# UBC-AWP/vision-sam3-yolo-lameless

Hardware: AMD Instinct MI355X
Metric: frames/sec (whole node) for YOLO+SAM3+DINOv3 feature extraction, 1080p clips (higher is better)
Workload: dtype f16; 1 GPU; BASELINE cfg#5, dense schedule: fused per-frame path on a synthetic 5 s @ 30 fps 1080p clip (150 unique BGR frames resident in HBM): YOLOv8-l detect (letterbox 384x640, NMS, scale_boxes; f16 plan) -> SAM (Hiera-B+ image encoder + FPN at 1024x1024, box-prompted mask decoder, 1080p mask + statistics + contour features) + DINOv3 ViT-L/16 embed (224x224) on EVERY frame; per-frame records packed, gathe; parallelism=one clip per GPU, 1 GPU(s), one gather per step, streams=7

## Files before the change

### vision-sam3-yolo-lameless_amd/csrc/pre.hip

```cpp
#include "common.h"

namespace {

constexpr int PRECISION_BITS = 32 - 8 - 2;

__device__ __forceinline__ uint8_t clip8(int v) {
  const int top = (256 << PRECISION_BITS) - 1;
  v = v < 0 ? 0 : (v > top ? top : v);
  return (uint8_t)((unsigned)v >> PRECISION_BITS);
}

__device__ __forceinline__ int tap(unsigned byte, int coef) { return __mul24((int)byte, coef); }

constexpr int RESIZE_H_MAX_ROW = 16384;
constexpr int RESIZE_H_LDS = 2 * RESIZE_H_MAX_ROW;
constexpr int RESIZE_H_ROWS = 4;

inline int resize_h_group(int rowb) {
  int r = (RESIZE_H_LDS - 16) / rowb;
  r = r > 8 ? 8 : r;
  return r >= RESIZE_H_ROWS ? r / RESIZE_H_ROWS * RESIZE_H_ROWS : r;
}

__global__ __launch_bounds__(256) void pil_resize_h_kernel(const uint8_t* __restrict__ src, uint8_t* __restrict__ dst,
                                                           int n, int sh, int sw, int dw, int group,
                                                           const int32_t* __restrict__ bounds,
                                                           const int32_t* __restrict__ kk, int ksize, int swap_rb) {
  __shared__ __attribute__((aligned(16))) uint8_t buf[RESIZE_H_LDS];
  const int rowb = sw * 3;
  const int64_t rows = (int64_t)n * sh;
  const int dwq = (dw + 3) & ~3;
  for (int64_t row0 = (int64_t)blockIdx.x * group; row0 < rows; row0 += (int64_t)gridDim.x * group) {
    const int nr = rows - row0 < group ? (int)(rows - row0) : group;
    const uint8_t* s0 = src + row0 * rowb;
    const int span = nr * rowb;
    const int mis = (int)(reinterpret_cast<uintptr_t>(s0) & 15);
    int head = mis ? 16 - mis : 0;
    head = head > span ? span : head;
    for (int i = threadIdx.x; i < head; i += blockDim.x) buf[mis + i] = s0[i];
    const int nvec = (span - head) / 16;
    for (int v = threadIdx.x; v < nvec; v += blockDim.x)
      *reinterpret_cast<u32x4*>(buf + mis + head + v * 16) = *reinterpret_cast<const u32x4*>(s0 + head + v * 16);
    for (int i = head + nvec * 16 + threadIdx.x; i < span; i += blockDim.x) buf[mis + i] = s0[i];
    __syncthreads();
    const int ntask = dwq * ((nr + RESIZE_H_ROWS - 1) / RESIZE_H_ROWS);
    for (int t0 = 0; t0 < ntask; t0 += blockDim.x) {
      const int t = t0 + threadIdx.x;
      const int rg = t / dwq, xq = t - rg * dwq;
      const int r0 = rg * RESIZE_H_ROWS;
      const bool live = t < ntask && xq < dw;
      const int xo = xq < dw ? xq : dw - 1;
      int rb[RESIZE_H_ROWS];
#pragma unroll
      for (int r = 0; r < RESIZE_H_ROWS; ++r) rb[r] = mis + (r0 + r < nr ? r0 + r : nr - 1) * rowb;
      const int xmin = bounds[2 * xo], cnt = bounds[2 * xo + 1];
      const int32_t* k = kk + (int64_t)xo * ksize;
      int a[RESIZE_H_ROWS][3];
#pragma unroll
      for (int r = 0; r < RESIZE_H_ROWS; ++r) a[r][0] = a[r][1] = a[r][2] = 1 << (PRECISION_BITS - 1);
      for (int x = 0; x < cnt; ++x) {
        const int c = k[x];
        const int off = (xmin + x) * 3;
#pragma unroll
        for (int r = 0; r < RESIZE_H_ROWS; ++r) {
          const uint8_t* s = buf + rb[r] + off;
          a[r][0] += tap(s[0], c);
          a[r][1] += tap(s[1], c);
          a[r][2] += tap(s[2], c);
        }
      }
      const int j = xq & 3;
      const bool quad = xq - j + 4 <= dw;
#pragma unroll
      for (int r = 0; r < RESIZE_H_ROWS; ++r) {
        const unsigned b0 = clip8(swap_rb ? a[r][2] : a[r][0]), b1 = clip8(a[r][1]), b2 = clip8(swap_rb ? a[r][0] : a[r][2]);
        const unsigned px = b0 | (b1 << 8) | (b2 << 16);
        const unsigned nx = __shfl_down(px, 1, 64);
        if (!live || r0 + r >= nr) continue;
        uint8_t* d = dst + (row0 + r0 + r) * dw * 3 + xq * 3;
        if (quad && ((reinterpret_cast<uintptr_t>(d) - 3 * j) & 3) == 0) {
          if (j < 3) *reinterpret_cast<unsigned*>(d - 3 * j + 4 * j) = (px >> (8 * j)) | (nx << (24 - 8 * j));
        } else {
          d[0] = (uint8_t)b0;
          d[1] = (uint8_t)b1;
          d[2] = (uint8_t)b2;
        }
      }
    }
    __syncthreads();
  }
}

__global__ __launch_bounds__(256) void pil_resize_v_kernel(const uint8_t* __restrict__ src, uint8_t* __restrict__ dst,
                                                           int n, int sh, int dh, int w,
                                                           const int32_t* __restrict__ bounds,
                                                           const int32_t* __restrict__ kk, int ksize) {
  const int rowb = w * 3;
  const int64_t total = (int64_t)n * dh * rowb;
  for (int64_t i = (int64_t)blockIdx.x * blockDim.x + threadIdx.x; i < total; i += (int64_t)gridDim.x * blockDim.x) {
    const int xb = (int)(i % rowb);
    const int64_t r = i / rowb;
    const int yo = (int)(r % dh);
    const int img = (int)(r / dh);
    const int ymin = bounds[2 * yo], cnt = bounds[2 * yo + 1];
    const int32_t* k = kk + (int64_t)yo * ksize;
    const uint8_t* s = src + ((int64_t)img * sh + ymin) * rowb + xb;
    int a = 1 << (PRECISION_BITS - 1);
    for (int y = 0; y < cnt; ++y) a += tap(s[(int64_t)y * rowb], k[y]);
    dst[i] = clip8(a);
  }
}

template <int DW>
__global__ __launch_bounds__(256) void pil_resize_vw_kernel(const uint8_t* __restrict__ src, uint8_t* __restrict__ dst, int n, int sh,
                                                            int dh, int w, const int32_t* __restrict__ bounds,
                                                            const int32_t* __restrict__ kk, int ksize) {
  typedef unsigned vec_t __attribute__((ext_vector_type(DW)));
  const int rowb = w * 3, roww = (rowb + 4 * DW - 1) / (4 * DW);
  const int64_t total = (int64_t)n * dh * roww;
  for (int64_t i = (int64_t)blockIdx.x * blockDim.x + threadIdx.x; i < total; i += (int64_t)gridDim.x * blockDim.x) {
    const int xw = (int)(i % roww);
    const int64_t r = i / roww;
    const int yo = (int)(r % dh);
    const int img = (int)(r / dh);
    const int ymin = bounds[2 * yo], cnt = bounds[2 * yo + 1];
    const int32_t* k = kk + (int64_t)yo * ksize;
    const int xb = xw * (4 * DW) + 4 * DW <= rowb ? xw * (4 * DW) : rowb - 4 * DW;
    const uint8_t* s = src + ((int64_t)img * sh + ymin) * rowb + xb;
    int a[4 * DW];
#pragma unroll
    for (int e = 0; e < 4 * DW; ++e) a[e] = 1 << (PRECISION_BITS - 1);
    for (int y = 0; y < cnt; ++y) {
      vec_t v;
      if (DW == 4)
        v = *reinterpret_cast<const vec_t*>(s + (int64_t)y * rowb);
      else
        __builtin_memcpy(&v, s + (int64_t)y * rowb, sizeof(v));
      const int c = k[y];
#pragma unroll
      for (int q = 0; q < DW; ++q) {
        a[4 * q + 0] += tap(v[q] & 255u, c);
        a[4 * q + 1] += tap((v[q] >> 8) & 255u, c);
        a[4 * q + 2] += tap((v[q] >> 16) & 255u, c);
        a[4 * q + 3] += tap(v[q] >> 24, c);
      }
    }
    vec_t o;
#pragma unroll
    for (int q = 0; q < DW; ++q)
      o[q] = (unsigned)clip8(a[4 * q]) | ((unsigned)clip8(a[4 * q + 1]) << 8) | ((unsigned)clip8(a[4 * q + 2]) << 16) |
             ((unsigned)clip8(a[4 * q + 3]) << 24);
    if (DW == 4)
      *reinterpret_cast<vec_t*>(dst + r * rowb + xb) = o;
    else
      __builtin_memcpy(dst + r * rowb + xb, &o, sizeof(o));
  }
}

__global__ __launch_bounds__(256) void patchify_norm_kernel(const uint8_t* __restrict__ img, half_t* __restrict__ out,
                                                            int n, int ih, int iw, int top, int left, int gh, int gw,
                                                            int P, int64_t ldo, const float* __restrict__ lut) {
  const int ch = gh * P, cw = gw * P;
  const int64_t total = (int64_t)n * ch * cw;
  for (int64_t i = (int64_t)blockIdx.x * blockDim.x + threadIdx.x; i < total; i += (int64_t)gridDim.x * blockDim.x) {
    const int x = (int)(i % cw);
    const int64_t r = i / cw;
    const int y = (int)(r % ch);
    const int b = (int)(r / ch);
    const uint8_t* s = img + (((int64_t)b * ih + top + y) * iw + left + x) * 3;
    const int py = y / P, ky = y - py * P, px = x / P, kx = x - px * P;
    half_t* d = out + (((int64_t)b * gh + py) * gw + px) * ldo + (ky * P + kx) * 3;
#pragma unroll
    for (int c = 0; c < 3; ++c) d[c] = (half_t)lut[c * 256 + s[c]];
  }
}

constexpr int FR_ROWS = 8;
constexpr int FR_COLS = 256;
constexpr int FR_MAX_LDS = 65536;

__global__ __launch_bounds__(FR_COLS) void float_resize_patchify_kernel(
    const uint8_t* __restrict__ src, half_t* __restrict__ out, int sh, int sw, int gh, int gw, int P, int64_t ldo,
    const int32_t* __restrict__ bh, const float* __restrict__ kh, int ksh, const int32_t* __restrict__ bv,
    const float* __restrict__ kv, int ksv, int seg_cols, float rescale, float m0, float m1, float m2, float s0, float s1,
    float s2, int swap_rb) {
  extern __shared__ __attribute__((aligned(16))) float seg[];
  const int tid = threadIdx.x;
  const int dh = gh * P, dw = gw * P;
  const int img = blockIdx.z;
  const int x0 = blockIdx.x * FR_COLS, xo = x0 + tid;
  const int y0 = blockIdx.y * FR_ROWS;
  const bool live = xo < dw;
  const int xl = (x0 + FR_COLS < dw ? x0 + FR_COLS : dw) - 1;
  int c_lo = bh[2 * x0];
  c_lo = c_lo < 0 ? 0 : (c_lo > sw ? sw : c_lo);
  int c_hi = bh[2 * xl] + bh[2 * xl + 1];
  c_hi = c_hi > sw ? sw : c_hi;
  if (c_hi > c_lo + seg_cols) c_hi = c_lo + seg_cols;
  if (c_hi < c_lo) c_hi = c_lo;
  int xmin = 0, xcnt = 0;
  if (live) {
    xmin = bh[2 * xo];
    xcnt = bh[2 * xo + 1];
    if (xmin < c_lo) xmin = c_lo;
    if (xcnt > ksh) xcnt = ksh;
    if (xcnt > c_hi - xmin) xcnt = c_hi - xmin;
    if (xcnt < 0) xcnt = 0;
  }
  const float* kx = kh + (int64_t)(live ? xo : 0) * ksh;
  int ymin[FR_ROWS], ycnt[FR_ROWS];
  int r_lo = sh, r_hi = 0;
#pragma unroll
  for (int r = 0; r < FR_ROWS; ++r) {
    ymin[r] = 0;
    ycnt[r] = 0;
    if (y0 + r < dh) {
      int a = bv[2 * (y0 + r)], c = bv[2 * (y0 + r) + 1];
      a = a < 0 ? 0 : a;
      c = c > ksv ? ksv : c;
      c = c > sh - a ? sh - a : c;
      c = c < 0 ? 0 : c;
      ymin[r] = a;
      ycnt[r] = c;
      if (c > 0) {
        r_lo = a < r_lo ? a : r_lo;
        r_hi = a + c > r_hi ? a + c : r_hi;
      }
    }
  }
  float acc[FR_ROWS][3];
#pragma unroll
  for (int r = 0; r < FR_ROWS; ++r) acc[r][0] = acc[r][1] = acc[r][2] = 0.f;

  const int nbytes = (c_hi - c_lo) * 3;
  for (int y = r_lo; y < r_hi; ++y) {
    const uint8_t* srow = src + (((int64_t)img * sh + y) * sw + c_lo) * 3;
    const int mis = (int)(reinterpret_cast<uintptr_t>(srow) & 15);
    int head = mis ? 16 - mis : 0;
    head = head > nbytes ? nbytes : head;
    const int pad = (4 - (head & 3)) & 3;
    float* s = seg + pad;
    if (tid < head) s[tid] = (float)srow[tid] * rescale;
    const int nvec = (nbytes - head) / 16;
    for (int v = tid; v < nvec; v += FR_COLS) {
      const u32x4 x = *reinterpret_cast<const u32x4*>(srow + head + v * 16);
      f32x4* d = reinterpret_cast<f32x4*>(s + head + v * 16);
#pragma unroll
      for (int q = 0; q < 4; ++q) {
        f32x4 f;
        f[0] = (float)(x[q] & 255u) * rescale;
        f[1] = (float)((x[q] >> 8) & 255u) * rescale;
        f[2] = (float)((x[q] >> 16) & 255u) * rescale;
        f[3] = (float)(x[q] >> 24) * rescale;
        d[q] = f;
      }
    }
    for (int i = head + nvec * 16 + tid; i < nbytes; i += FR_COLS) s[i] = (float)srow[i] * rescale;
    __syncthreads();
    float h0 = 0.f, h1 = 0.f, h2 = 0.f;
    const float* p = s + (xmin - c_lo) * 3;
    for (int j = 0; j < xcnt; ++j) {
      const float w = kx[j];
      h0 = __builtin_fmaf(p[3 * j + 0], w, h0);
      h1 = __builtin_fmaf(p[3 * j + 1], w, h1);
      h2 = __builtin_fmaf(p[3 * j + 2], w, h2);
    }
#pragma unroll
    for (int r = 0; r < FR_ROWS; ++r) {
      if (y >= ymin[r] && y < ymin[r] + ycnt[r]) {
        const float w = kv[(int64_t)(y0 + r) * ksv + (y - ymin[r])];
        acc[r][0] = __builtin_fmaf(h0, w, acc[r][0]);
        acc[r][1] = __builtin_fmaf(h1, w, acc[r][1]);
        acc[r][2] = __builtin_fmaf(h2, w, acc[r][2]);
      }
    }
    __syncthreads();
  }
  if (!live) return;
  const int px = xo / P, kxp = xo - px * P;
#pragma unroll
  for (int r = 0; r < FR_ROWS; ++r) {
    const int yo = y0 + r;
    if (yo >= dh) break;
    const int py = yo / P, ky = yo - py * P;
    half_t* d = out + (((int64_t)img * gh + py) * gw + px) * ldo + (ky * P + kxp) * 3;
    d[0] = (half_t)(((swap_rb ? acc[r][2] : acc[r][0]) - m0) / s0);
    d[1] = (half_t)((acc[r][1] - m1) / s1);
    d[2] = (half_t)(((swap_rb ? acc[r][0] : acc[r][2]) - m2) / s2);
  }
}

inline int grid_for(int64_t total) {
  int64_t g = (total + 255) / 256;
  if (g > 256 * 8) g = 256 * 8;
  if (g < 1) g = 1;
  return (int)g;
}

}

extern "C" int lmx_k_pil_resize_h(const uint8_t* src, uint8_t* dst, int n, int sh, int sw, int dw, const int32_t* bounds,
                                  const int32_t* kk, int ksize, int swap_rb, lmx_stream_t stream) {
  LMX_REQUIRE(src && dst && bounds && kk, "lmx_k_pil_resize_h: null pointer");
  LMX_REQUIRE(n > 0 && sh > 0 && sw > 0 && dw > 0 && ksize > 0, "lmx_k_pil_resize_h: shape");
  LMX_REQUIRE(sw * 3 <= RESIZE_H_MAX_ROW, "lmx_k_pil_resize_h: source rows wider than %d pixels are not staged", RESIZE_H_MAX_ROW / 3);
  const int group = resize_h_group(sw * 3);
  const int64_t groups = ((int64_t)n * sh + group - 1) / group;
  hipLaunchKernelGGL(pil_resize_h_kernel, dim3((unsigned)(groups < 256 * 16 ? groups : 256 * 16)), dim3(256), 0,
                     reinterpret_cast<hipStream_t>(stream), src, dst, n, sh, sw, dw, group, bounds, kk, ksize, swap_rb);
  return lmx_launch_check("pil_resize_h_kernel");
}

extern "C" int lmx_k_pil_resize_v(const uint8_t* src, uint8_t* dst, int n, int sh, int dh, int w, const int32_t* bounds,
                                  const int32_t* kk, int ksize, lmx_stream_t stream) {
  LMX_REQUIRE(src && dst && bounds && kk, "lmx_k_pil_resize_v: null pointer");
  LMX_REQUIRE(n > 0 && sh > 0 && dh > 0 && w > 0 && ksize > 0, "lmx_k_pil_resize_v: shape");
  const uintptr_t al = (uintptr_t)src | (uintptr_t)dst | (uintptr_t)(w * 3);
  if ((al & 15) == 0) {
    hipLaunchKernelGGL(pil_resize_vw_kernel<4>, dim3(grid_for((int64_t)n * dh * (w * 3 / 16))), dim3(256), 0,
                       reinterpret_cast<hipStream_t>(stream), src, dst, n, sh, dh, w, bounds, kk, ksize);
    return lmx_launch_check("pil_resize_vw_kernel<4>");
  }
  if (w * 3 >= 4) {
    hipLaunchKernelGGL(pil_resize_vw_kernel<1>, dim3(grid_for((int64_t)n * dh * ((w * 3 + 3) / 4))), dim3(256), 0,
                       reinterpret_cast<hipStream_t>(stream), src, dst, n, sh, dh, w, bounds, kk, ksize);
    return lmx_launch_check("pil_resize_vw_kernel<1>");
  }
  hipLaunchKernelGGL(pil_resize_v_kernel, dim3(grid_for((int64_t)n * dh * w * 3)), dim3(256), 0,
                     reinterpret_cast<hipStream_t>(stream), src, dst, n, sh, dh, w, bounds, kk, ksize);
  return lmx_launch_check("pil_resize_v_kernel");
}

extern "C" int lmx_k_float_resize_patchify(const uint8_t* src, void* out, int n, int sh, int sw, int gh, int gw, int P,
                                           int64_t ldo, const int32_t* bounds_h, const float* kk_h, int ksize_h,
                                           const int32_t* bounds_v, const float* kk_v, int ksize_v, int seg_cols,
                                           float rescale, const float* mean_std, int swap_rb, lmx_stream_t stream) {
  LMX_REQUIRE(src && out && bounds_h && kk_h && bounds_v && kk_v && mean_std, "lmx_k_float_resize_patchify: null pointer");
  LMX_REQUIRE(n > 0 && n <= 65535 && sh > 0 && sw > 0 && gh > 0 && gw > 0 && P > 0 && ksize_h > 0 && ksize_v > 0,
              "lmx_k_float_resize_patchify: shape");
  LMX_REQUIRE(ldo >= (int64_t)P * P * 3, "lmx_k_float_resize_patchify: ldo %lld < P*P*3", (long long)ldo);
  LMX_REQUIRE((int64_t)gh * P <= 65535 * (int64_t)FR_ROWS && (int64_t)gw * P <= (1 << 20), "lmx_k_float_resize_patchify: output size");
  LMX_REQUIRE(seg_cols > 0 && seg_cols <= sw, "lmx_k_float_resize_patchify: seg_cols %d outside 1..%d", seg_cols, sw);
  const int64_t lds = ((int64_t)seg_cols * 3 + 4) * (int64_t)sizeof(float);
  LMX_REQUIRE(lds <= FR_MAX_LDS, "lmx_k_float_resize_patchify: a tile of %d output columns reads %d source columns; more than %d are not staged",
              FR_COLS, seg_cols, (FR_MAX_LDS / 4 - 4) / 3);
  LMX_REQUIRE(mean_std[3] != 0.f && mean_std[4] != 0.f && mean_std[5] != 0.f, "lmx_k_float_resize_patchify: zero std");
  const dim3 grid((unsigned)((gw * P + FR_COLS - 1) / FR_COLS), (unsigned)((gh * P + FR_ROWS - 1) / FR_ROWS), (unsigned)n);
  hipLaunchKernelGGL(float_resize_patchify_kernel, grid, dim3(FR_COLS), (size_t)lds, reinterpret_cast<hipStream_t>(stream), src,
                     reinterpret_cast<half_t*>(out), sh, sw, gh, gw, P, ldo, bounds_h, kk_h, ksize_h, bounds_v, kk_v, ksize_v,
                     seg_cols, rescale, mean_std[0], mean_std[1], mean_std[2], mean_std[3], mean_std[4], mean_std[5], swap_rb);
  return lmx_launch_check("float_resize_patchify_kernel");
}

extern "C" int lmx_k_patchify_norm(const uint8_t* img, void* out, int n, int ih, int iw, int top, int left, int gh,
                                   int gw, int P, int64_t ldo, const float* lut, lmx_stream_t stream) {
  LMX_REQUIRE(img && out && lut, "lmx_k_patchify_norm: null pointer");
  LMX_REQUIRE(n > 0 && gh > 0 && gw > 0 && P > 0 && ldo >= (int64_t)P * P * 3, "lmx_k_patchify_norm: shape");
  LMX_REQUIRE(top >= 0 && left >= 0 && top + gh * P <= ih && left + gw * P <= iw,
              "lmx_k_patchify_norm: crop (%d,%d)+(%d,%d) outside %dx%d", top, left, gh * P, gw * P, ih, iw);
  hipLaunchKernelGGL(patchify_norm_kernel, dim3(grid_for((int64_t)n * gh * P * gw * P)), dim3(256), 0,
                     reinterpret_cast<hipStream_t>(stream), img, reinterpret_cast<half_t*>(out), n, ih, iw, top, left, gh,
                     gw, P, ldo, lut);
  return lmx_launch_check("patchify_norm_kernel");
}
```

### vision-sam3-yolo-lameless_amd/csrc/yolo.hip

```cpp
#include "common.h"

namespace {

inline int grid_for(int64_t total, int block = 256) {
  int64_t g = (total + block - 1) / block;
  if (g > 256 * 8) g = 256 * 8;
  if (g < 1) g = 1;
  return (int)g;
}

__global__ __launch_bounds__(256) void letterbox_kernel(const uint8_t* __restrict__ src, uint8_t* __restrict__ dst, int n,
                                                        int sh, int sw, int rh, int rw, int top, int left, int oh, int ow,
                                                        const int* __restrict__ xofs, const short* __restrict__ ialpha,
                                                        const int* __restrict__ yofs, const short* __restrict__ ibeta,
                                                        int swap_rb, int identity) {
  const int64_t total = (int64_t)n * oh * ow;
  for (int64_t i = (int64_t)blockIdx.x * blockDim.x + threadIdx.x; i < total; i += (int64_t)gridDim.x * blockDim.x) {
    const int ox = (int)(i % ow);
    const int64_t r = i / ow;
    const int oy = (int)(r % oh);
    const int img = (int)(r / oh);
    uint8_t* d = dst + i * 3;
    const int dy = oy - top, dx = ox - left;
    if (dy < 0 || dy >= rh || dx < 0 || dx >= rw) {
      d[0] = d[1] = d[2] = 114;
      continue;
    }
    uint8_t v[3];
    const uint8_t* S = src + (int64_t)img * sh * sw * 3;
    if (identity) {
      const uint8_t* s = S + ((int64_t)dy * sw + dx) * 3;
      v[0] = s[0];
      v[1] = s[1];
      v[2] = s[2];
    } else {
      const int sx0 = xofs[dx];
      const int sx1 = sx0 + 1 < sw ? sx0 + 1 : sw - 1;
      const int a0 = ialpha[2 * dx], a1 = ialpha[2 * dx + 1];
      int sy0 = yofs[dy], sy1 = yofs[dy] + 1;
      sy0 = sy0 < 0 ? 0 : (sy0 < sh ? sy0 : sh - 1);
      sy1 = sy1 < 0 ? 0 : (sy1 < sh ? sy1 : sh - 1);
      const int b0 = ibeta[2 * dy], b1 = ibeta[2 * dy + 1];
      const uint8_t* r0 = S + (int64_t)sy0 * sw * 3;
      const uint8_t* r1 = S + (int64_t)sy1 * sw * 3;
#pragma unroll
      for (int c = 0; c < 3; ++c) {
        const int h0 = (int)r0[sx0 * 3 + c] * a0 + (int)r0[sx1 * 3 + c] * a1;
        const int h1 = (int)r1[sx0 * 3 + c] * a0 + (int)r1[sx1 * 3 + c] * a1;
        const int val = (((b0 * (h0 >> 4)) >> 16) + ((b1 * (h1 >> 4)) >> 16) + 2) >> 2;
        v[c] = (uint8_t)(val < 0 ? 0 : (val > 255 ? 255 : val));
      }
    }
    if (swap_rb) {
      d[0] = v[2];
      d[1] = v[1];
      d[2] = v[0];
    } else {
      d[0] = v[0];
      d[1] = v[1];
      d[2] = v[2];
    }
  }
}

template <int CO_T>
__global__ __launch_bounds__(256) void stem_conv_kernel(const uint8_t* __restrict__ img, const float* __restrict__ w,
                                                        const float* __restrict__ bias, half_t* __restrict__ out, int n,
                                                        int H, int W, int Ho, int Wo, int Cout) {
  extern __shared__ __attribute__((aligned(16))) char smem[];
  float* ws = reinterpret_cast<float*>(smem);
  for (int i = threadIdx.x; i < 27 * Cout; i += blockDim.x) ws[i] = w[i];
  for (int i = threadIdx.x; i < Cout; i += blockDim.x) ws[27 * Cout + i] = bias[i];
  __syncthreads();
  const int64_t total = (int64_t)n * Ho * Wo;
  for (int64_t i = (int64_t)blockIdx.x * blockDim.x + threadIdx.x; i < total; i += (int64_t)gridDim.x * blockDim.x) {
    const int ox = (int)(i % Wo);
    const int64_t r = i / Wo;
    const int oy = (int)(r % Ho);
    const int b = (int)(r / Ho);
    float x[27];
#pragma unroll
    for (int ky = 0; ky < 3; ++ky)
#pragma unroll
      for (int kx = 0; kx < 3; ++kx) {
        const int iy = oy * 2 - 1 + ky, ix = ox * 2 - 1 + kx;
        const bool ok = (unsigned)iy < (unsigned)H && (unsigned)ix < (unsigned)W;
        const uint8_t* s = img + (((int64_t)b * H + (ok ? iy : 0)) * W + (ok ? ix : 0)) * 3;
#pragma unroll
        for (int c = 0; c < 3; ++c) x[(ky * 3 + kx) * 3 + c] = ok ? (float)s[c] / 255.0f : 0.0f;
      }
    half_t* o = out + i * Cout;
    for (int c0 = 0; c0 < Cout; c0 += CO_T) {
      float acc[CO_T];
#pragma unroll
      for (int j = 0; j < CO_T; ++j) acc[j] = ws[27 * Cout + c0 + j];
#pragma unroll
      for (int t = 0; t < 27; ++t) {
        const float xv = x[t];
#pragma unroll
        for (int j = 0; j < CO_T; ++j) acc[j] = fmaf(xv, ws[t * Cout + c0 + j], acc[j]);
      }
      half8_t hv;
#pragma unroll
      for (int j = 0; j < CO_T; ++j) {
        const float v = acc[j] / (1.0f + expf(-acc[j]));
        hv[j] = (half_t)v;
      }
      *reinterpret_cast<half8_t*>(o + c0) = hv;
    }
  }
}

__global__ __launch_bounds__(256) void maxpool5_kernel(const half_t* __restrict__ src, int64_t lds, half_t* __restrict__ dst,
                                                       int64_t ldd, int n, int H, int W, int C) {
  const int cc = C / 8;
  const int64_t total = (int64_t)n * H * W * cc;
  for (int64_t i = (int64_t)blockIdx.x * blockDim.x + threadIdx.x; i < total; i += (int64_t)gridDim.x * blockDim.x) {
    const int c = (int)(i % cc) * 8;
    const int64_t p = i / cc;
    const int x = (int)(p % W);
    const int64_t r = p / W;
    const int y = (int)(r % H);
    const int b = (int)(r / H);
    half8_t m;
#pragma unroll
    for (int e = 0; e < 8; ++e) m[e] = (half_t)(-65504.0f);
    for (int dy = -2; dy <= 2; ++dy) {
      const int yy = y + dy;
      if ((unsigned)yy >= (unsigned)H) continue;
      for (int dx = -2; dx <= 2; ++dx) {
        const int xx = x + dx;
        if ((unsigned)xx >= (unsigned)W) continue;
        const half8_t v = *reinterpret_cast<const half8_t*>(src + (((int64_t)b * H + yy) * W + xx) * lds + c);
#pragma unroll
        for (int e = 0; e < 8; ++e) m[e] = v[e] > m[e] ? v[e] : m[e];
      }
    }
    *reinterpret_cast<half8_t*>(dst + p * ldd + c) = m;
  }
}

__global__ __launch_bounds__(256) void upsample2_kernel(const half_t* __restrict__ src, int64_t lds, half_t* __restrict__ dst,
                                                        int64_t ldd, int n, int H, int W, int C) {
  const int cc = C / 8;
  const int Ho = 2 * H, Wo = 2 * W;
  const int64_t total = (int64_t)n * Ho * Wo * cc;
  for (int64_t i = (int64_t)blockIdx.x * blockDim.x + threadIdx.x; i < total; i += (int64_t)gridDim.x * blockDim.x) {
    const int c = (int)(i % cc) * 8;
    const int64_t p = i / cc;
    const int x = (int)(p % Wo);
    const int64_t r = p / Wo;
    const int y = (int)(r % Ho);
    const int b = (int)(r / Ho);
    *reinterpret_cast<half8_t*>(dst + p * ldd + c) =
        *reinterpret_cast<const half8_t*>(src + (((int64_t)b * H + (y >> 1)) * W + (x >> 1)) * lds + c);
  }
}

__global__ __launch_bounds__(256) void detect_decode_kernel(const float* __restrict__ head, float* __restrict__ pred, int n,
                                                            int H, int W, int nc, int ch, float stride, int a_off,
                                                            int A) {
  const int64_t total = (int64_t)n * H * W * 4;
  for (int64_t i0 = (int64_t)blockIdx.x * blockDim.x; i0 < total; i0 += (int64_t)gridDim.x * blockDim.x) {
    const int64_t i = i0 + threadIdx.x;
    const bool live = i < total;
    const int side = (int)(i & 3);
    const int64_t cell = live ? (i >> 2) : 0;
    const int x = (int)(cell % W);
    const int64_t r = cell / W;
    const int y = (int)(r % H);
    const int b = (int)(r / H);
    const float* hrow = head + cell * ch;
    float l[16];
    float mx = -INFINITY;
#pragma unroll
    for (int k = 0; k < 4; ++k) {
      const f32x4 v = *reinterpret_cast<const f32x4*>(hrow + side * 16 + k * 4);
#pragma unroll
      for (int e = 0; e < 4; ++e) {
        l[k * 4 + e] = v[e];
        mx = fmaxf(mx, v[e]);
      }
    }
    float se = 0.f;
#pragma unroll
    for (int k = 0; k < 16; ++k) {
      l[k] = expf(l[k] - mx);
      se += l[k];
    }
    float dist = 0.f;
#pragma unroll
    for (int k = 0; k < 16; ++k) dist += (l[k] / se) * (float)k;
    const int base = threadIdx.x & ~3;
    const float dl = __shfl(dist, (base & 63) + 0, 64), dt = __shfl(dist, (base & 63) + 1, 64);
    const float dr = __shfl(dist, (base & 63) + 2, 64), db = __shfl(dist, (base & 63) + 3, 64);
    if (!live) continue;
    float* prow = pred + ((int64_t)b * A + a_off + (int64_t)y * W + x) * (4 + nc);
    if (side == 0) {
      const float ax = (float)x + 0.5f, ay = (float)y + 0.5f;
      const float x1 = ax - dl, y1 = ay - dt, x2 = ax + dr, y2 = ay + db;
      prow[0] = ((x1 + x2) / 2.f) * stride;
      prow[1] = ((y1 + y2) / 2.f) * stride;
      prow[2] = (x2 - x1) * stride;
      prow[3] = (y2 - y1) * stride;
    }
    const float* hc = hrow + 64;
    float* pc = prow + 4;
    const bool al = (reinterpret_cast<uintptr_t>(pc) & 15) == 0;
    const int nc4 = nc & ~3;
    for (int c = side * 4; c < nc4; c += 16) {
      const f32x4 v = *reinterpret_cast<const f32x4*>(hc + c);
      f32x4 s;
#pragma unroll
      for (int e = 0; e < 4; ++e) s[e] = 1.0f / (1.0f + expf(-v[e]));
      if (al) {
        *reinterpret_cast<f32x4*>(pc + c) = s;
      } else {
#pragma unroll
        for (int e = 0; e < 4; ++e) pc[c + e] = s[e];
      }
    }
    for (int c = nc4 + side; c < nc; c += 4) pc[c] = 1.0f / (1.0f + expf(-hc[c]));
  }
}

__global__ __launch_bounds__(256) void scale_boxes_kernel(float* __restrict__ boxes, int total, float padx, float pady,
                                                          float gain, float w, float h) {
  const int i = blockIdx.x * blockDim.x + threadIdx.x;
  if (i >= total) return;
  float* b = boxes + (int64_t)i * 4;
  float x1 = (b[0] - padx) / gain, y1 = (b[1] - pady) / gain, x2 = (b[2] - padx) / gain, y2 = (b[3] - pady) / gain;
  b[0] = fminf(fmaxf(x1, 0.f), w);
  b[1] = fminf(fmaxf(y1, 0.f), h);
  b[2] = fminf(fmaxf(x2, 0.f), w);
  b[3] = fminf(fmaxf(y2, 0.f), h);
}

struct PoseLevels {
  const float* raw[3];
  int h[3], w[3], off[3];
  float stride[3];
};
__global__ __launch_bounds__(256) void pose_gather_kernel(const PoseLevels L, int64_t ldk, const int* __restrict__ src,
                                                          const int* __restrict__ counts, int n, int max_det, int K, int ndim,
                                                          float padx, float pady, float gain, float fw, float fh,
                                                          float* __restrict__ out) {
  const int64_t total = (int64_t)n * max_det * K;
  for (int64_t i = (int64_t)blockIdx.x * blockDim.x + threadIdx.x; i < total; i += (int64_t)gridDim.x * blockDim.x) {
    const int k = (int)(i % K);
    const int64_t r = i / K;
    const int j = (int)(r % max_det);
    const int b = (int)(r / max_det);
    float* o = out + i * ndim;
    if (j >= counts[b]) {
      for (int e = 0; e < ndim; ++e) o[e] = 0.f;
      continue;
    }
    const int a = src[(int64_t)b * max_det + j];
    const int l = a >= L.off[2] ? 2 : (a >= L.off[1] ? 1 : 0);
    const int local = a - L.off[l];
    const int y = local / L.w[l], x = local - y * L.w[l];
    const float* v = L.raw[l] + (((int64_t)b * L.h[l] + y) * L.w[l] + x) * ldk + k * ndim;
    const float X = (v[0] * 2.0f + (float)x) * L.stride[l];
    const float Y = (v[1] * 2.0f + (float)y) * L.stride[l];
    o[0] = fminf(fmaxf((X - padx) / gain, 0.f), fw);
    o[1] = fminf(fmaxf((Y - pady) / gain, 0.f), fh);
    if (ndim == 3) o[2] = 1.0f / (1.0f + expf(-v[2]));
  }
}

}

extern "C" int lmx_k_pose_gather(const float* raw0, const float* raw1, const float* raw2, int64_t ldk, const int32_t* hw,
                                 const float* strides, const int32_t* src, const int32_t* counts, int n, int max_det, int K,
                                 int ndim, float padx, float pady, float gain, float w, float h, float* out,
                                 lmx_stream_t stream) {
  LMX_REQUIRE(raw0 && raw1 && raw2 && hw && strides && src && counts && out, "lmx_k_pose_gather: null pointer");
  LMX_REQUIRE(n > 0 && max_det > 0 && K > 0 && (ndim == 2 || ndim == 3) && ldk >= (int64_t)K * ndim && gain > 0.f,
              "lmx_k_pose_gather: arguments");
  PoseLevels L;
  L.raw[0] = raw0;
  L.raw[1] = raw1;
  L.raw[2] = raw2;
  int off = 0;
  for (int l = 0; l < 3; ++l) {
    LMX_REQUIRE(hw[2 * l] > 0 && hw[2 * l + 1] > 0, "lmx_k_pose_gather: level %d geometry", l);
    L.h[l] = hw[2 * l];
    L.w[l] = hw[2 * l + 1];
    L.off[l] = off;
    L.stride[l] = strides[l];
    off += L.h[l] * L.w[l];
  }
  hipLaunchKernelGGL(pose_gather_kernel, dim3(grid_for((int64_t)n * max_det * K)), dim3(256), 0,
                     reinterpret_cast<hipStream_t>(stream), L, ldk, src, counts, n, max_det, K, ndim, padx, pady, gain, w, h, out);
  return lmx_launch_check("pose_gather_kernel");
}

extern "C" int lmx_k_letterbox(const uint8_t* src, uint8_t* dst, int n, int sh, int sw, int rh, int rw, int top, int left,
                               int oh, int ow, const int32_t* xofs, const int16_t* ialpha, const int32_t* yofs,
                               const int16_t* ibeta, int swap_rb, lmx_stream_t stream) {
  LMX_REQUIRE(src && dst, "lmx_k_letterbox: null pointer");
  LMX_REQUIRE(n > 0 && sh > 0 && sw > 0 && rh > 0 && rw > 0 && oh >= top + rh && ow >= left + rw && top >= 0 && left >= 0,
              "lmx_k_letterbox: geometry");
  const int identity = (rh == sh && rw == sw) ? 1 : 0;
  LMX_REQUIRE(identity || (xofs && ialpha && yofs && ibeta), "lmx_k_letterbox: null tables");
  hipLaunchKernelGGL(letterbox_kernel, dim3(grid_for((int64_t)n * oh * ow)), dim3(256), 0,
                     reinterpret_cast<hipStream_t>(stream), src, dst, n, sh, sw, rh, rw, top, left, oh, ow, xofs, ialpha, yofs,
                     ibeta, swap_rb, identity);
  return lmx_launch_check("letterbox_kernel");
}

extern "C" int lmx_k_stem_conv(const uint8_t* img, const float* w, const float* bias, void* out, int n, int H, int W, int Cout,
                               lmx_stream_t stream) {
  LMX_REQUIRE(img && w && bias && out, "lmx_k_stem_conv: null pointer");
  LMX_REQUIRE(n > 0 && H > 0 && W > 0 && Cout > 0 && Cout % 8 == 0 && Cout <= 256, "lmx_k_stem_conv: shape (Cout %d)", Cout);
  LMX_REQUIRE(aligned16(out), "lmx_k_stem_conv: out alignment");
  const int Ho = (H + 2 - 3) / 2 + 1, Wo = (W + 2 - 3) / 2 + 1;
  const size_t smem = (size_t)28 * Cout * sizeof(float);
  hipLaunchKernelGGL((stem_conv_kernel<8>), dim3(grid_for((int64_t)n * Ho * Wo)), dim3(256), smem,
                     reinterpret_cast<hipStream_t>(stream), img, w, bias, reinterpret_cast<half_t*>(out), n, H, W, Ho, Wo, Cout);
  return lmx_launch_check("stem_conv_kernel");
}

extern "C" int lmx_k_maxpool5(const void* src, int64_t lds, void* dst, int64_t ldd, int n, int H, int W, int C,
                              lmx_stream_t stream) {
  LMX_REQUIRE(src && dst, "lmx_k_maxpool5: null pointer");
  LMX_REQUIRE(n > 0 && H > 0 && W > 0 && C > 0 && C % 8 == 0 && lds % 8 == 0 && ldd % 8 == 0 && lds >= C && ldd >= C,
              "lmx_k_maxpool5: shape");
  LMX_REQUIRE(aligned16(src) && aligned16(dst), "lmx_k_maxpool5: alignment");
  hipLaunchKernelGGL(maxpool5_kernel, dim3(grid_for((int64_t)n * H * W * (C / 8))), dim3(256), 0,
                     reinterpret_cast<hipStream_t>(stream), reinterpret_cast<const half_t*>(src), lds,
                     reinterpret_cast<half_t*>(dst), ldd, n, H, W, C);
  return lmx_launch_check("maxpool5_kernel");
}

extern "C" int lmx_k_upsample2(const void* src, int64_t lds, void* dst, int64_t ldd, int n, int H, int W, int C,
                               lmx_stream_t stream) {
  LMX_REQUIRE(src && dst, "lmx_k_upsample2: null pointer");
  LMX_REQUIRE(n > 0 && H > 0 && W > 0 && C > 0 && C % 8 == 0 && lds % 8 == 0 && ldd % 8 == 0 && lds >= C && ldd >= C,
              "lmx_k_upsample2: shape");
  LMX_REQUIRE(aligned16(src) && aligned16(dst), "lmx_k_upsample2: alignment");
  hipLaunchKernelGGL(upsample2_kernel, dim3(grid_for((int64_t)n * 4 * H * W * (C / 8))), dim3(256), 0,
                     reinterpret_cast<hipStream_t>(stream), reinterpret_cast<const half_t*>(src), lds,
                     reinterpret_cast<half_t*>(dst), ldd, n, H, W, C);
  return lmx_launch_check("upsample2_kernel");
}

extern "C" int lmx_k_detect_decode(const float* head, int64_t ldh, float* pred, int n, int H, int W, int nc, float stride,
                                   int a_off, int A, lmx_stream_t stream) {
  LMX_REQUIRE(head && pred, "lmx_k_detect_decode: null pointer");
  LMX_REQUIRE(n > 0 && H > 0 && W > 0 && nc > 0 && a_off >= 0 && a_off + H * W <= A, "lmx_k_detect_decode: shape");
  LMX_REQUIRE(ldh >= 64 + nc && ldh % 4 == 0 && aligned16(head), "lmx_k_detect_decode: head row stride %lld", (long long)ldh);
  hipLaunchKernelGGL(detect_decode_kernel, dim3(grid_for((int64_t)n * H * W * 4)), dim3(256), 0,
                     reinterpret_cast<hipStream_t>(stream), head, pred, n, H, W, nc, (int)ldh, stride, a_off, A);
  return lmx_launch_check("detect_decode_kernel");
}

extern "C" int lmx_k_scale_boxes(float* boxes, int total, float padx, float pady, float gain, float w, float h,
                                 lmx_stream_t stream) {
  LMX_REQUIRE(boxes && total > 0 && gain > 0.f, "lmx_k_scale_boxes: arguments");
  hipLaunchKernelGGL(scale_boxes_kernel, dim3((total + 255) / 256), dim3(256), 0, reinterpret_cast<hipStream_t>(stream), boxes,
                     total, padx, pady, gain, w, h);
  return lmx_launch_check("scale_boxes_kernel");
}
```

Before: 818.8 frames/s.

## Use MFMA for YOLO stem conv and word-wise LDS reads in PIL horizontal resize

Adds an MFMA-based (16x16x4 f32) stem convolution kernel for Cout of 16, 32 or 64. Each wavefront computes 16 pixels against all output channels, with the next pixel group's input gathered ahead of use (software prefetch) and SiLU fused into the output store. The PIL horizontal resize now reads LDS as 32-bit words realigned with alignbyte and processes four taps per iteration instead of byte loads. Its global-to-LDS staging is also batched into registers before the LDS writes. It also adds debug-only compile paths (LMX_DBG_H_*) and a larger LDS slack, at the cost of extra register pressure and more complex code.

```diff
diff --git a/vision-sam3-yolo-lameless_amd/csrc/pre.hip b/vision-sam3-yolo-lameless_amd/csrc/pre.hip
--- a/vision-sam3-yolo-lameless_amd/csrc/pre.hip
+++ b/vision-sam3-yolo-lameless_amd/csrc/pre.hip
@@ -14,10 +14,12 @@
 
 constexpr int RESIZE_H_MAX_ROW = 16384;
 constexpr int RESIZE_H_LDS = 2 * RESIZE_H_MAX_ROW;
+constexpr int RESIZE_H_SLACK = 32;
 constexpr int RESIZE_H_ROWS = 4;
+constexpr int RESIZE_H_VEC = RESIZE_H_LDS / 16 / 256;
 
 inline int resize_h_group(int rowb) {
-  int r = (RESIZE_H_LDS - 16) / rowb;
+  int r = (RESIZE_H_LDS - RESIZE_H_SLACK) / rowb;
   r = r > 8 ? 8 : r;
   return r >= RESIZE_H_ROWS ? r / RESIZE_H_ROWS * RESIZE_H_ROWS : r;
 }
@@ -27,6 +29,7 @@
                                                            const int32_t* __restrict__ bounds,
                                                            const int32_t* __restrict__ kk, int ksize, int swap_rb) {
   __shared__ __attribute__((aligned(16))) uint8_t buf[RESIZE_H_LDS];
+  const unsigned* bufw = reinterpret_cast<const unsigned*>(buf);
   const int rowb = sw * 3;
   const int64_t rows = (int64_t)n * sh;
   const int dwq = (dw + 3) & ~3;
@@ -39,8 +42,13 @@
     head = head > span ? span : head;
     for (int i = threadIdx.x; i < head; i += blockDim.x) buf[mis + i] = s0[i];
     const int nvec = (span - head) / 16;
-    for (int v = threadIdx.x; v < nvec; v += blockDim.x)
-      *reinterpret_cast<u32x4*>(buf + mis + head + v * 16) = *reinterpret_cast<const u32x4*>(s0 + head + v * 16);
+    u32x4 pre[RESIZE_H_VEC];
+#pragma unroll
+    for (int i = 0; i < RESIZE_H_VEC; ++i)
+      if ((int)threadIdx.x + 256 * i < nvec) pre[i] = *reinterpret_cast<const u32x4*>(s0 + head + (threadIdx.x + 256 * i) * 16);
+#pragma unroll
+    for (int i = 0; i < RESIZE_H_VEC; ++i)
+      if ((int)threadIdx.x + 256 * i < nvec) *reinterpret_cast<u32x4*>(buf + mis + head + (threadIdx.x + 256 * i) * 16) = pre[i];
     for (int i = head + nvec * 16 + threadIdx.x; i < span; i += blockDim.x) buf[mis + i] = s0[i];
     __syncthreads();
     const int ntask = dwq * ((nr + RESIZE_H_ROWS - 1) / RESIZE_H_ROWS);
@@ -50,25 +58,54 @@
       const int r0 = rg * RESIZE_H_ROWS;
       const bool live = t < ntask && xq < dw;
       const int xo = xq < dw ? xq : dw - 1;
-      int rb[RESIZE_H_ROWS];
-#pragma unroll
-      for (int r = 0; r < RESIZE_H_ROWS; ++r) rb[r] = mis + (r0 + r < nr ? r0 + r : nr - 1) * rowb;
       const int xmin = bounds[2 * xo], cnt = bounds[2 * xo + 1];
+      int a[RESIZE_H_ROWS][3];
+      unsigned ad[RESIZE_H_ROWS];
+#pragma unroll
+      for (int r = 0; r < RESIZE_H_ROWS; ++r) {
+        a[r][0] = a[r][1] = a[r][2] = 1 << (PRECISION_BITS - 1);
+        ad[r] = mis + (r0 + r < nr ? r0 + r : nr - 1) * rowb + xmin * 3;
+      }
+#if defined(LMX_DBG_H_STAGEONLY)
+#pragma unroll
+      for (int r = 0; r < RESIZE_H_ROWS; ++r) a[r][0] += cnt + (int)bufw[ad[r] >> 2];
+#else
       const int32_t* k = kk + (int64_t)xo * ksize;
-      int a[RESIZE_H_ROWS][3];
-#pragma unroll
-      for (int r = 0; r < RESIZE_H_ROWS; ++r) a[r][0] = a[r][1] = a[r][2] = 1 << (PRECISION_BITS - 1);
+#if defined(LMX_DBG_H_ONEREAD)
+      unsigned one[RESIZE_H_ROWS];
+#pragma unroll
+      for (int r = 0; r < RESIZE_H_ROWS; ++r) one[r] = bufw[ad[r] >> 2];
       for (int x = 0; x < cnt; ++x) {
         const int c = k[x];
-        const int off = (xmin + x) * 3;
 #pragma unroll
         for (int r = 0; r < RESIZE_H_ROWS; ++r) {
-          const uint8_t* s = buf + rb[r] + off;
-          a[r][0] += tap(s[0], c);
-          a[r][1] += tap(s[1], c);
-          a[r][2] += tap(s[2], c);
+          const unsigned w = one[r] + x;
+          a[r][0] += tap(w & 255, c);
+          a[r][1] += tap((w >> 8) & 255, c);
+          a[r][2] += tap((w >> 16) & 255, c);
         }
       }
+#else
+      unsigned lo[RESIZE_H_ROWS];
+#pragma unroll
+      for (int r = 0; r < RESIZE_H_ROWS; ++r) lo[r] = bufw[ad[r] >> 2];
+      for (int x = 0; x < cnt; x += 4) {
+        const int c0 = k[x], c1 = x + 1 < cnt ? k[x + 1] : 0, c2 = x + 2 < cnt ? k[x + 2] : 0, c3 = x + 3 < cnt ? k[x + 3] : 0;
+#pragma unroll
+        for (int r = 0; r < RESIZE_H_ROWS; ++r) {
+          const unsigned* p = bufw + (ad[r] >> 2) + (x >> 2) * 3;
+          const unsigned d1 = p[1], d2 = p[2], d3 = p[3];
+          const unsigned ph = ad[r] & 3;
+          const unsigned w0 = __builtin_amdgcn_alignbyte(d1, lo[r], ph), w1 = __builtin_amdgcn_alignbyte(d2, d1, ph),
+                         w2 = __builtin_amdgcn_alignbyte(d3, d2, ph);
+          lo[r] = d3;
+          a[r][0] += tap(w0 & 255, c0) + tap(w0 >> 24, c1) + tap((w1 >> 16) & 255, c2) + tap((w2 >> 8) & 255, c3);
+          a[r][1] += tap((w0 >> 8) & 255, c0) + tap(w1 & 255, c1) + tap(w1 >> 24, c2) + tap((w2 >> 16) & 255, c3);
+          a[r][2] += tap((w0 >> 16) & 255, c0) + tap((w1 >> 8) & 255, c1) + tap(w2 & 255, c2) + tap(w2 >> 24, c3);
+        }
+      }
+#endif
+#endif
       const int j = xq & 3;
       const bool quad = xq - j + 4 <= dw;
 #pragma unroll
diff --git a/vision-sam3-yolo-lameless_amd/csrc/yolo.hip b/vision-sam3-yolo-lameless_amd/csrc/yolo.hip
--- a/vision-sam3-yolo-lameless_amd/csrc/yolo.hip
+++ b/vision-sam3-yolo-lameless_amd/csrc/yolo.hip
@@ -60,6 +60,98 @@
       d[1] = v[1];
       d[2] = v[2];
     }
+  }
+}
+
+template <int NT>
+__device__ __forceinline__ int stem_chan(int ct, int i) {
+  return NT == 1 ? i : (ct >> 1) * 32 + (i >> 2) * 8 + (ct & 1) * 4 + (i & 3);
+}
+
+template <int NT>
+__global__ __launch_bounds__(256) void stem_conv_mfma_kernel(const uint8_t* __restrict__ img, const float* __restrict__ w,
+                                                             const float* __restrict__ bias, half_t* __restrict__ out,
+                                                             int total, int H, int W, int Ho, int Wo) {
+  constexpr int Cout = 16 * NT;
+  __shared__ float xtab[257];
+  for (int i = threadIdx.x; i < 256; i += blockDim.x) xtab[i] = (float)(uint8_t)i / 255.0f;
+  if (threadIdx.x == 0) xtab[256] = 0.0f;
+  __syncthreads();
+  const int lane = threadIdx.x & 63, p16 = lane & 15, q = lane >> 4;
+  float wa[NT][7];
+  f32x4 bi[NT];
+#pragma unroll
+  for (int ct = 0; ct < NT; ++ct) {
+#pragma unroll
+    for (int s = 0; s < 7; ++s) wa[ct][s] = 4 * s + q < 27 ? w[(4 * s + q) * Cout + stem_chan<NT>(ct, p16)] : -0.0f;
+#pragma unroll
+    for (int r = 0; r < 4; ++r) bi[ct][r] = bias[stem_chan<NT>(ct, q * 4 + r)];
+  }
+  int ky[7], kx[7], koff[7];
+#pragma unroll
+  for (int s = 0; s < 7; ++s) {
+    const int t = 4 * s + q;
+    ky[s] = t < 27 ? t / 9 : 1 << 20;
+    kx[s] = t % 9 / 3;
+    koff[s] = t < 27 ? (ky[s] * W + kx[s]) * 3 + t % 3 : 0;
+  }
+  const int groups = (total + 15) / 16;
+  const int nw = gridDim.x * (blockDim.x >> 6);
+  auto fetch = [&](int g, int (&u)[7]) {
+    const int pix = g * 16 + p16;
+    const bool valid = g < groups && pix < total;
+    const int pc = valid ? pix : 0;
+    const int ox = pc % Wo, r = pc / Wo;
+    const int oy = r % Ho, b = r / Ho;
+    const int iy0 = oy * 2 - 1, ix0 = ox * 2 - 1;
+    const int64_t base = (((int64_t)b * H + iy0) * W + ix0) * 3;
+#pragma unroll
+    for (int s = 0; s < 7; ++s) {
+      const bool ok = valid && (unsigned)(iy0 + ky[s]) < (unsigned)H && (unsigned)(ix0 + kx[s]) < (unsigned)W;
+      const int v = img[ok ? base + koff[s] : 0];
+      u[s] = ok ? v : 256;
+    }
+  };
+  int g = blockIdx.x * (blockDim.x >> 6) + (threadIdx.x >> 6);
+  int u[7], un[7];
+  fetch(g, u);
+  for (; g < groups; g += nw) {
+    float x[7];
+#pragma unroll
+    for (int s = 0; s < 7; ++s) x[s] = xtab[u[s]];
+    fetch(g + nw, un);
+    f32x4 acc[NT];
+#pragma unroll
+    for (int ct = 0; ct < NT; ++ct) acc[ct] = bi[ct];
+#pragma unroll
+    for (int s = 0; s < 7; ++s)
+#pragma unroll
+      for (int ct = 0; ct < NT; ++ct) acc[ct] = __builtin_amdgcn_mfma_f32_16x16x4f32(wa[ct][s], x[s], acc[ct], 0, 0, 0);
+    half_t h[NT][4];
+#pragma unroll
+    for (int ct = 0; ct < NT; ++ct)
+#pragma unroll
+      for (int r = 0; r < 4; ++r) {
+        const float a = acc[ct][r];
+        h[ct][r] = (half_t)(a / (1.0f + expf(-a)));
+      }
+    const int pix = g * 16 + p16;
+    if (pix < total) {
+      half_t* o = out + (int64_t)pix * Cout;
+      if constexpr (NT == 1) {
+        half4_t hv = {h[0][0], h[0][1], h[0][2], h[0][3]};
+        *reinterpret_cast<half4_t*>(o + q * 4) = hv;
+      } else {
+#pragma unroll
+        for (int c2 = 0; c2 < NT / 2; ++c2) {
+          half8_t hv = {h[2 * c2][0],     h[2 * c2][1],     h[2 * c2][2],     h[2 * c2][3],
+                        h[2 * c2 + 1][0], h[2 * c2 + 1][1], h[2 * c2 + 1][2], h[2 * c2 + 1][3]};
+          *reinterpret_cast<half8_t*>(o + c2 * 32 + q * 8) = hv;
+        }
+      }
+    }
+#pragma unroll
+    for (int s = 0; s < 7; ++s) u[s] = un[s];
   }
 }
 
@@ -316,6 +408,21 @@
   LMX_REQUIRE(n > 0 && H > 0 && W > 0 && Cout > 0 && Cout % 8 == 0 && Cout <= 256, "lmx_k_stem_conv: shape (Cout %d)", Cout);
   LMX_REQUIRE(aligned16(out), "lmx_k_stem_conv: out alignment");
   const int Ho = (H + 2 - 3) / 2 + 1, Wo = (W + 2 - 3) / 2 + 1;
+  const int64_t total = (int64_t)n * Ho * Wo;
+  if ((Cout == 16 || Cout == 32 || Cout == 64) && total <= INT32_MAX - 16) {
+    const int64_t wgs = ((total + 15) / 16 + 3) / 4;
+    const dim3 grid((unsigned)(wgs < 256 * 8 ? wgs : 256 * 8));
+    const hipStream_t st = reinterpret_cast<hipStream_t>(stream);
+    half_t* o = reinterpret_cast<half_t*>(out);
+    const int tot = (int)total;
+    if (Cout == 64)
+      hipLaunchKernelGGL((stem_conv_mfma_kernel<4>), grid, dim3(256), 0, st, img, w, bias, o, tot, H, W, Ho, Wo);
+    else if (Cout == 32)
+      hipLaunchKernelGGL((stem_conv_mfma_kernel<2>), grid, dim3(256), 0, st, img, w, bias, o, tot, H, W, Ho, Wo);
+    else
+      hipLaunchKernelGGL((stem_conv_mfma_kernel<1>), grid, dim3(256), 0, st, img, w, bias, o, tot, H, W, Ho, Wo);
+    return lmx_launch_check("stem_conv_kernel");
+  }
   const size_t smem = (size_t)28 * Cout * sizeof(float);
   hipLaunchKernelGGL((stem_conv_kernel<8>), dim3(grid_for((int64_t)n * Ho * Wo)), dim3(256), smem,
                      reinterpret_cast<hipStream_t>(stream), img, w, bias, reinterpret_cast<half_t*>(out), n, H, W, Ho, Wo, Cout);
```

New measurement: 822.2 frames/s, median of 6. Within noise of the previous version (+0.4%).
